# JoshuaQSH/FALCON-TTDforGNNs

Hardware: AMD Instinct MI355X
Metric: tt_embedding_lookups_per_sec (higher is better)
Workload: dtype f32; 1 GPU; ogbn-products TTEmbeddingBag fwd+bwd+SGD per step, frontier of a 2048-seed batch = 409600 unique uniform ids per GPU, bag length 1; num_embeddings=2449029, ids_per_gpu_step=409600, parallelism=dp1

## Files before the change

### falcon-ttdforgnns_amd/csrc/ttemb_api.hip

```cpp
#include "ttemb_common.h"
#include "ttemb_cache.h"

#include <dlfcn.h>

#include <atomic>
#include <cstdarg>
#include <cstdio>
#include <cstdlib>
#include <cstring>

namespace ttemb {

static thread_local char g_err[512] = "";
static std::atomic<int> g_path{TTEMB_PATH_AUTO};

int fail(int code, const char* fmt, ...) {
  va_list ap;
  va_start(ap, fmt);
  vsnprintf(g_err, sizeof(g_err), fmt, ap);
  va_end(ap);
  return code;
}

int check_hip(hipError_t e, const char* what) {
// ... 930 lines not shown

extern "C" {

int ttemb_abi_version(void) { return TTEMB_ABI_VERSION; }

const char* ttemb_last_error(void) { return g_err; }

int ttemb_set_path(int32_t path) {
  if (path < TTEMB_PATH_AUTO || path > TTEMB_PATH_PER_BAG) return fail(TTEMB_E_BADARG, "unknown path %d", path);
  g_path.store(path);
  return TTEMB_OK;
}

int ttemb_set_piece_limits(int64_t rows, int64_t ids) {
  fast3_set_piece_limits(rows, ids);
  return TTEMB_OK;
}

int ttemb_set_wide_slab_min_ids(int64_t ids) {
  fast3_set_wide_slab_min_ids(ids);
  return TTEMB_OK;
}

int ttemb_grouping_layout(const ttemb_shape_t* shape, int64_t nnz, int64_t* out) {
  if (shape == nullptr || out == nullptr || nnz < 0) return fail(TTEMB_E_BADARG, "grouping_layout: bad argument");
  DevShape ds;
  int rc = make_dev_shape(shape, &ds);
  if (rc) return rc;
  return fast3_grouping_layout(ds, nnz, out);
}

int ttemb_set_spin_limit(int64_t tries) {
  fast3_set_spin_limit(tries);
  return TTEMB_OK;
}

int ttemb_init(void) { return fault_word_init(); }

int ttemb_status(void) {
  if (g_fault_state.load(std::memory_order_acquire) == 0) (void)fault_word_init();
  return pending_device_fault();
}

int ttemb_profile_enable(int32_t on) {
  if (on != 0)
    for (int i = 0; i < kProfSlots; ++i) g_prof_valid[i] = false;
// ... 653 lines not shown
```

### falcon-ttdforgnns_amd/csrc/ttemb_common.h

```cpp
#pragma once

#include <hip/hip_runtime.h>
#include <stdint.h>

#include <atomic>

#include "../../include/ttemb.h"

namespace ttemb {

constexpr int kWave = 64;
constexpr int kMaxProbes = 3;
constexpr int64_t kEmptyKey = -1;

struct DevShape {
  int T;
  int p[TTEMB_MAX_CORES];
  int q[TTEMB_MAX_CORES];
  int R[TTEMB_MAX_CORES + 1];
  long long L[TTEMB_MAX_CORES];
  int D;
  int row_len[TTEMB_MAX_CORES];
  int part_len[TTEMB_MAX_CORES];
  int part_max;
// ... 19 lines not shown
};
int allow_big_lds(const void* kernel, size_t lds_bytes, LdsGate* gate, const char* what);
int device_cus();

int64_t generic_fwd_lds_bytes(const DevShape& s);
int64_t generic_bwd_lds_bytes(const DevShape& s);
int launch_forward_generic(const DevShape& s, const CorePtrs& cores, const int64_t* indices,
                           const int64_t* rowidx, const int64_t* offsets, int64_t B, int64_t nnz,
                           const int32_t* nnz_dev, float* output, hipStream_t st);
int launch_backward_generic(const DevShape& s, const CorePtrs& cores, const int64_t* indices,
                            const int64_t* rowidx, const int64_t* offsets, int64_t B, int64_t nnz,
                            const int32_t* nnz_dev, const float* d_output, const CorePtrsMut& d_cores, hipStream_t st);
int launch_zero_cores(const DevShape& s, const CorePtrsMut& d_cores, hipStream_t st);

bool fast3_supported(const DevShape& s);
bool fast3_pays(const DevShape& s, int64_t nnz);
bool fast3_prefix_in_chain(const DevShape& s, int64_t nnz, int64_t B);
bool fast3_group_products_in_chain(const DevShape& s, int64_t nnz, int64_t B);
bool fast3_fits(const DevShape& s, int64_t nnz, int64_t B);
bool fast3_fits_in_pieces(const DevShape& s, int64_t nnz, int64_t B);
void fast3_set_piece_limits(int64_t rows, int64_t ids);
int fast3_grouping_layout(const DevShape& s, int64_t nnz, int64_t* out);
void fast3_set_spin_limit(int64_t tries);
void fast3_set_wide_slab_min_ids(int64_t ids);
uint32_t* fault_word(hipStream_t st);
int fault_word_init();
int pending_device_fault();
int64_t fast3_workspace_bytes(const DevShape& s, int32_t op, int64_t nnz, int64_t B);
int64_t fast3_plan_bytes(const DevShape& s, int64_t nnz);
int launch_forward_fast3(const DevShape& s, const CorePtrs& cores, const int64_t* indices,
                         const int64_t* rowidx, const int64_t* offsets, int64_t nnz,
                         const int32_t* nnz_dev, int64_t B, float* output, bool zero_rows, void* ws,
                         int64_t ws_bytes, void* plan, int64_t plan_bytes, int phase, hipStream_t st, void* header);
constexpr int64_t kFast3HeaderBytes = 40960;
struct FusedUpdateK {
  float* w[TTEMB_MAX_CORES];
  float* st[TTEMB_MAX_CORES];
  float lr, eps;
  const float* lr_dev;
  float* v[TTEMB_MAX_CORES];
  uint32_t* step;
  float b1, omb1, b2, omb2;
  float wd;
  int32_t decoupled;
  uint32_t* poison_out;
  int32_t sticky;
// ... 128 lines not shown
```

### falcon-ttdforgnns_amd/csrc/ttemb_fast3.hip

```cpp
#include "ttemb_common.h"
#include "ttemb_cache.h"

#include <atomic>
#include <cstdlib>
#include <cstring>



namespace ttemb {

typedef float f32x4 __attribute__((ext_vector_type(4)));


constexpr int kChunk = 16;
constexpr uint32_t kMultiBit = 0x80000000u;

template <int Q0, int Q1, int Q2, int R1, int R2>
struct Cfg {
  static constexpr int M2 = Q0 * Q1;
  static constexpr int MT2 = (M2 + 15) / 16;
  static constexpr int KS1 = R1 / 4;
  static constexpr int KS2 = R2 / 4;
  static constexpr int N1 = Q1 * R2;
  static constexpr int NT1 = (N1 + 15) / 16;
// ... 2113 lines not shown
      if constexpr (SHARED) {
        for (int e0 = 0; e0 < ROW2; e0 += kWave) {
          const int e = e0 + lane, src = (e >> 2) & 63;
          const float x = __shfl(acc[n].x, src, kWave), y = __shfl(acc[n].y, src, kWave);
          const float z = __shfl(acc[n].z, src, kWave), w = __shfl(acc[n].w, src, kWave);
          const float v = (e & 3) == 0 ? x : ((e & 3) == 1 ? y : ((e & 3) == 2 ? z : w));
          if (e < ROW2) atomicAdd(slab + (size_t)i2 * stride + e, v);
        }
      } else {
        if (lane < F4) *reinterpret_cast<float4*>(slab + (size_t)i2 * stride + 4 * lane) = acc[n];
      }
    }
  }
}

#ifndef TTEMB_EPI_SLICES
#define TTEMB_EPI_SLICES 16
#endif
constexpr int kEpiSlices = TTEMB_EPI_SLICES;
__device__ __forceinline__ bool sparse_groups(const GroupPlan& plan, uint32_t G) {
  return __builtin_amdgcn_readfirstlane(plan.counts[G]) * 4u < 3u * G;
}

template <int Q0, int Q1, int Q2, int R1, int R2>
struct EpiCfg {
  static constexpr int G1_BYTES = R1 * (Q1 * R2 + 1) * 4;
#ifndef TTEMB_EPI_SHARE_BYTES
#define TTEMB_EPI_SHARE_BYTES (8 * 1024)
#endif
  static constexpr int WAVES = G1_BYTES > TTEMB_EPI_SHARE_BYTES ? 4 : 1;
};

template <int Q0, int Q1, int Q2, int R1, int R2, bool SKIP>
__device__ __forceinline__ void epilogue_unit(
    const float* __restrict__ G0, const float* __restrict__ G1, uint32_t p0, uint32_t p1, uint32_t gpw, const GroupPlan& plan,
    float* dpbuf, float* g1buf, uint32_t slice, uint32_t slices, uint32_t i1) {
  using C = Cfg<Q0, Q1, Q2, R1, R2>;
  constexpr int GM = 16 / Q0;
  constexpr int LDD = C::N1 + 4;
  constexpr int PF = C::M2 * R2;
  constexpr int BF4 = 16 * C::N1 / 4;
  constexpr int NLB = (BF4 + kWave - 1) / kWave;
  constexpr int KS3 = C::N1 / 4;
  static_assert(C::N1 % 4 == 0, "dP rows move as float4");
  constexpr int EW = EpiCfg<Q0, Q1, Q2, R1, R2>::WAVES;
  const int lane = threadIdx.x & 63;
  const int hi = lane >> 4, lo = lane & 15;
  const bool active = slice < slices;
  const uint32_t i0_begin = active ? slice * gpw : p0;
  const uint32_t i0_end = i0_begin + gpw < p0 ? i0_begin + gpw : p0;
  const uint32_t g_begin = i1 * p0 + (active ? i0_begin : 0u);
  const uint32_t G = p0 * p1;
  const rsrc_t r_dp = make_rsrc(plan.dptab, G * (uint32_t)PF * 4u);
  const rsrc_t r_g0 = make_rsrc(G0, p0 * (uint32_t)C::ROW0 * 4u);
  const rsrc_t r_part = make_rsrc(plan.g0part, G * (uint32_t)C::ROW0 * 4u);

  f32x4 g1acc[C::RT1][C::NT1];
#pragma unroll
  for (int t = 0; t < C::RT1; ++t)
#pragma unroll
    for (int nt = 0; nt < C::NT1; ++nt) g1acc[t][nt] = (f32x4){0.f, 0.f, 0.f, 0.f};

  const uint32_t cnt_l = (i0_begin + lane < i0_end) ? plan.counts[g_begin + lane] : 0u;
  const unsigned long long live = __ballot(cnt_l != 0);
  float4 nxt[NLB];
  float nxt_g0[4][C::RT1];
  auto request = [&](uint32_t k0) {
#pragma unroll
    for (int it = 0; it < NLB; ++it) {
      const int e = it * kWave + lane;
      const uint32_t gi = k0 + (uint32_t)(4 * e / PF);
      const bool on = (BF4 % kWave == 0 || e < BF4) && 4 * e / PF < GM && gi < gpw && ((live >> gi) & 1ull);
      nxt[it] = buf_load4(r_dp, on ? (g_begin + k0) * (uint32_t)(PF * 4) + 16u * e : kOob);
    }
#pragma unroll
    for (int s = 0; s < 4; ++s) {
      const int rho = 4 * s + hi;
      const uint32_t gi = k0 + (uint32_t)(rho / Q0);
      const bool on = rho / Q0 < GM && gi < gpw && ((live >> gi) & 1ull);
#pragma unroll
      for (int t = 0; t < C::RT1; ++t)
        nxt_g0[s][t] = __uint_as_float(buf_load1u(
            r_g0, (on && 16 * t + lo < R1) ? (i0_begin + gi) * (uint32_t)(C::ROW0 * 4) + 4u * ((rho % Q0) * R1 + 16 * t + lo) : kOob));
    }
  };
  auto next_live = [&](uint32_t k) {
    if constexpr (SKIP) {
      while (k < gpw && !((live >> k) & ((1ull << GM) - 1ull))) k += GM;
    }
    return k;
  };
  if constexpr (SKIP) {
    if (active && lane == 0) plan.epi_live[(size_t)slice * p1 + i1] = live != 0ull ? 1u : 0u;
    if (EW == 1 && live == 0ull) return;
  }
  const uint32_t k_first = next_live(0);
  request(k_first);
  {
    const float* g1 = G1 + (size_t)i1 * C::ROW1;
    constexpr int NG1 = (C::ROW1 + EW * kWave - 1) / (EW * kWave);
    const int t0 = (int)threadIdx.x;
    float g1v[NG1];
#pragma unroll
    for (int it = 0; it < NG1; ++it) {
      const int e = it * EW * kWave + t0;
      g1v[it] = (C::ROW1 % (EW * kWave) == 0 || e < C::ROW1) ? g1[e] : 0.f;
    }
#pragma unroll
    for (int it = 0; it < NG1; ++it) {
      const int e = it * EW * kWave + t0;
      if (C::ROW1 % (EW * kWave) == 0 || e < C::ROW1) g1buf[(e / C::N1) * C::LDG + e % C::N1] = g1v[it];
    }
    if constexpr (EW > 1) {
      __syncthreads();
      if (!active || (SKIP && live == 0ull)) return;
    }
  }
  const uint32_t n_here = i0_end - i0_begin;
  for (uint32_t k0 = k_first; k0 < n_here;) {
    float g0v[4][C::RT1];
#pragma unroll
    for (int it = 0; it < NLB; ++it) {
      const int e = it * kWave + lane;
      if (BF4 % kWave == 0 || e < BF4) *reinterpret_cast<float4*>(dpbuf + (4 * e / C::N1) * LDD + (4 * e) % C::N1) = nxt[it];
    }
#pragma unroll
    for (int s = 0; s < 4; ++s)
#pragma unroll
      for (int t = 0; t < C::RT1; ++t) g0v[s][t] = nxt_g0[s][t];
    __builtin_amdgcn_sched_barrier(0);
    const uint32_t k_next = next_live(k0 + GM);
    request(k_next);
    __builtin_amdgcn_fence(__ATOMIC_RELEASE, "wavefront");
    __builtin_amdgcn_wave_barrier();
    __builtin_amdgcn_fence(__ATOMIC_ACQUIRE, "wavefront");
    float b1[4][C::NT1];
#pragma unroll
    for (int s = 0; s < 4; ++s)
// ... 20 lines not shown
    f32x4 g0part[4][C::RT1];
#pragma unroll
    for (int c = 0; c < 4; ++c)
#pragma unroll
      for (int t = 0; t < C::RT1; ++t) g0part[c][t] = (f32x4){0.f, 0.f, 0.f, 0.f};
#pragma unroll
    for (int s = 0; s < KS3; ++s)
#pragma unroll
      for (int t = 0; t < C::RT1; ++t)
        g0part[s & 3][t] = __builtin_amdgcn_mfma_f32_16x16x4f32(a3[s], b3[s][t], g0part[s & 3][t], 0, 0, 0);
#pragma unroll
    for (int t = 0; t < C::RT1; ++t) {
      const f32x4 sum = (g0part[0][t] + g0part[1][t]) + (g0part[2][t] + g0part[3][t]);
#pragma unroll
      for (int r = 0; r < 4; ++r) {
        const int rho = 4 * hi + r;
        const uint32_t gi = k0 + (uint32_t)(rho / Q0);
        const bool on = rho / Q0 < GM && gi < n_here && 16 * t + lo < R1;
        buf_store1(r_part, on ? (g_begin + gi) * (uint32_t)(C::ROW0 * 4) + 4u * ((rho % Q0) * R1 + 16 * t + lo) : kOob, sum[r]);
      }
    }
    k0 = k_next;
  }
  float* dst = plan.g1part + ((size_t)slice * p1 + i1) * C::ROW1;
#pragma unroll
  for (int t = 0; t < C::RT1; ++t)
#pragma unroll
    for (int nt = 0; nt < C::NT1; ++nt)
#pragma unroll
      for (int r = 0; r < 4; ++r) {
        const int c = 16 * t + 4 * hi + r;
        if (c < R1 && (C::N1 % 16 == 0 || 16 * nt + lo < C::N1)) dst[c * C::N1 + 16 * nt + lo] = g1acc[t][nt][r];
      }
}

template <int Q0, int Q1, int Q2, int R1, int R2>
__global__ __launch_bounds__((EpiCfg<Q0, Q1, Q2, R1, R2>::WAVES * 64)) void fast3_group_epilogue_kernel(
    const float* __restrict__ G0, const float* __restrict__ G1, uint32_t p0, uint32_t p1, uint32_t gpw, uint32_t slices, GroupPlan plan,
    AdamPrep adam) {
  using C = Cfg<Q0, Q1, Q2, R1, R2>;
  constexpr int EW = EpiCfg<Q0, Q1, Q2, R1, R2>::WAVES;
  if (adam.step != nullptr && blockIdx.x == 0 && threadIdx.x == 0) adam_prepare(adam);
  __shared__ __attribute__((aligned(16))) float dpbuf_all[EW][16 * (C::N1 + 4)];
  __shared__ __attribute__((aligned(16))) float g1buf[R1 * C::LDG];
  const uint32_t wave = threadIdx.x >> 6;
  float* dpbuf = dpbuf_all[wave];
  const uint32_t nsb = (slices + EW - 1u) / EW;
  const uint32_t i1_blk = blockIdx.x / nsb;
  const uint32_t slice = (blockIdx.x - i1_blk * nsb) * EW + wave;
  if (sparse_groups(plan, p0 * p1))
    epilogue_unit<Q0, Q1, Q2, R1, R2, true>(G0, G1, p0, p1, gpw, plan, dpbuf, g1buf, slice, slices, i1_blk);
  else
    epilogue_unit<Q0, Q1, Q2, R1, R2, false>(G0, G1, p0, p1, gpw, plan, dpbuf, g1buf, slice, slices, i1_blk);
}

__device__ __forceinline__ void finalize_emit(const FusedUpdateK& upd, const AdamCoef& ac, float lr, int t, float* __restrict__ grad, int idx, float g) {
  if (upd.w[0] == nullptr) {
    grad[idx] = upd.eps != 0.f ? grad[idx] + g : g;
  } else if (upd.st[0] == nullptr) {
    upd.w[t][idx] -= lr * g;
  } else if (upd.v[0] != nullptr) {
    float w = upd.w[t][idx], m = upd.st[t][idx], v = upd.v[t][idx];
    adam_element(w, m, v, g, ac, lr, upd.eps, upd.b1, upd.omb1, upd.b2, upd.omb2, upd.wd, upd.decoupled);
    upd.st[t][idx] = m;
    upd.v[t][idx] = v;
    upd.w[t][idx] = w;
  } else {
    const float s2 = upd.st[t][idx] + g * g;
    upd.st[t][idx] = s2;
    upd.w[t][idx] -= lr * g / (sqrtf(s2) + upd.eps);
  }
}

__global__ __launch_bounds__(256) void fast3_finalize_kernel(GroupPlan plan, int tiles, int slices, int p0, int p1,
                                                             int g2_floats, int row0, int g1_floats, int q2, int r2,
                                                             float* __restrict__ dG0, float* __restrict__ dG1,
// ... 377 lines not shown
  const int64_t least = forced > 0 ? forced : (int64_t)8 * wide_slab_shares(s) * s.p[2];
  return nnz >= least;
}
static int64_t slab_count(const DevShape& s, int64_t nnz) {
  if (wide_slab(s, nnz)) return wide_slab_shares(s);
  return fused_dg2(s) ? fused_tiles(s, nnz) : (shared_slab(s) ? 1 : reduce_tiles(nnz));
}
static int epi_groups_per_wave(const DevShape& s) {
  int gpw = (s.p[0] + kEpiSlices - 1) / kEpiSlices;
  return gpw < 1 ? 1 : (gpw > 64 ? 64 : gpw);
}
static int wide_k_chunk(const DevShape& s) {
  const int64_t tiles = (int64_t)(s.R[1] / 64) * (s.q[1] * s.R[2] / 64) * s.p[1];
  int64_t parts = (4096 + tiles - 1) / tiles;
  parts = parts < 1 ? 1 : (parts > 8 ? 8 : parts);
  const int64_t K = (int64_t)s.p[0] * s.q[0];
  return (int)(((K + parts - 1) / parts + 31) / 32 * 32);
}
static int64_t wide_rows_stride(const DevShape& s) { return ((int64_t)s.p[0] * s.q[0] + 63) / 64 * 64 + 64; }
static int epi_slices(const DevShape& s) {
  if (wide(s)) return (int)(((int64_t)s.p[0] * s.q[0] + wide_k_chunk(s) - 1) / wide_k_chunk(s));
  const int g = epi_groups_per_wave(s);
  return (s.p[0] + g - 1) / g;
}

static int64_t max_chunks(const DevShape& s, int64_t nnz) {
  const int64_t G = num_groups(s);
  return nnz / kChunk + (nnz < G ? nnz : G) + 1;
}

int64_t fast3_plan_bytes(const DevShape& s, int64_t nnz) {
  const int64_t G = num_groups(s);
  return 2 * align256(nnz * 4) + align256((G + 1) * 4) + align256((G + 3) * 8) + align256(max_chunks(s, nnz) * 16) +
         align256(G * (int64_t)s.q[0] * s.q[1] * s.R[2] * 4);
}

static void carve_plan_part(const DevShape& s, int64_t nnz, char* base, GroupPlan* pl) {
  const int64_t G = num_groups(s);
  pl->i2s = (uint32_t*)base;
  base += align256(nnz * 4);
  pl->vals = (uint32_t*)base;
  base += align256(nnz * 4);
  pl->counts = (uint32_t*)base;
  base += align256((G + 1) * 4);
  pl->gpre = (uint64_t*)base;
  base += align256((G + 3) * 8);
// ... 422 lines not shown
#endif
    rc = run_wide_gemm<true, true, 1>(g, s, plan, st, "wide3_gemm_kernel (dG0)");
    if (rc) return rc;
  }
  {
    const int g2_floats = s.p[2] * C::ROW2, g1_floats = s.p[1] * C::ROW1;
    const int wgs = (g2_floats + 31) / 32 + (s.p[0] * C::ROW0 + 31) / 32 + (g1_floats + 1023) / 1024;
    hipLaunchKernelGGL(fast3_finalize_kernel, dim3((unsigned)wgs), dim3(256), 0, st, plan, (int)slab_count(s, nnz), epi_slices(s), s.p[0], s.p[1],
                       g2_floats, (int)C::ROW0, g1_floats, Q2, R2, d_cores.c[0], d_cores.c[1], d_cores.c[2], upd, 1);
  }
  profile_end(1, st);
  return check_hip(hipGetLastError(), "fast3_finalize_kernel (wide)");
}

#ifndef TTEMB_GFUSE_IDS
#define TTEMB_GFUSE_IDS -1
#endif
constexpr int64_t kGFuseIdsPerGroup = TTEMB_GFUSE_IDS;
template <int Q0, int Q1, int Q2, int R1, int R2>
struct GFuseCfg {
  using C = Cfg<Q0, Q1, Q2, R1, R2>;
  static constexpr bool ok = 16 / Q0 >= 2 && C::N1 % 16 == 0 && Q1 > 1;
};
static int64_t gfuse_limit(const DevShape& s) {
  if (kGFuseIdsPerGroup >= 0) return kGFuseIdsPerGroup;
  return s.R[2] >= 32 ? (int64_t(1) << 40) : (s.q[0] == 8 ? 16 : 8);
}

static bool gfuse_pays(const DevShape& s, int64_t nnz) {
  if (gfuse_limit(s) <= 0 || !classify(s) || fused_dg2(s)) return false;
  bool ok = false;
#define TTEMB_X(a, b, c, d, e) if (shape_is(s, a, b, c, d, e)) ok = GFuseCfg<a, b, c, d, e>::ok;
  TTEMB_FAST3_SHAPES(TTEMB_X)
#undef TTEMB_X
  const int64_t G = num_groups(s);
  return ok && (gfuse_limit(s) >= (int64_t(1) << 40) || nnz < gfuse_limit(s) * G) && (uint64_t)G * (uint64_t)s.p[0] < (uint64_t(1) << 40);
}
bool fast3_group_products_in_chain(const DevShape& s, int64_t nnz, int64_t B) { return fits_piece(s, nnz, B) && gfuse_pays(s, nnz); }

template <int Q0, int Q1, int Q2, int R1, int R2>
static int run_backward(const DevShape& s, const CorePtrs& cores, const GroupPlan& plan, int64_t nnz, int64_t B,
                        const float* d_output, const CorePtrsMut& d_cores, const FusedUpdate& upd, hipStream_t st) {
  using C = Cfg<Q0, Q1, Q2, R1, R2>;
  const int64_t G = num_groups(s);
  profile_begin(1, st);
  int rc;
  constexpr size_t wave_lds = (size_t)(C::PB_FLOATS + C::BB2_FLOATS + C::OB_FLOATS) * sizeof(float);
// ... 54 lines not shown
                       (uint32_t)G, (uint32_t)s.p[2], (uint32_t)nnz, d_output, (uint32_t)(B * s.D * 4), plan, GroupFuse{});
    profile_end(2, st);
    rc = check_hip(hipGetLastError(), "fast3_bwd_chunk_kernel");
    if (rc) return rc;
  }
  const int tiles = (int)reduce_tiles(nnz);
  const size_t reduce_lds = (size_t)(2 * s.p[2] + 1) * 4 + kRowsB * 2;
  const AdamPrep no_adam{nullptr, 0.0, 0.0};
  const AdamPrep reduce_adam = gfuse ? adam_prep_of(upd) : no_adam, epi_adam = gfuse ? no_adam : adam_prep_of(upd);
  if (fused) {
  } else if (shared_slab(s)) {
    rc = launch_zero(plan.g2part, (size_t)s.p[2] * C::ROW2 * 4, st, "zero the shared dG2 slab");
    if (rc) return rc;
    hipLaunchKernelGGL((fast3_dg2_reduce_kernel<C::ROW2, kRowsB, NWB, true>), dim3((unsigned)tiles), dim3(NWB * 64), reduce_lds, st,
                       plan, (int)G, (uint32_t)s.p[2], (uint32_t)reduce_rows(nnz), (uint32_t)C::ROW2, reduce_adam);

  } else {
    hipLaunchKernelGGL((fast3_dg2_reduce_kernel<C::ROW2, kRowsB, NWB, false>), dim3((unsigned)tiles), dim3(NWB * 64), reduce_lds, st,
                       plan, (int)G, (uint32_t)s.p[2], (uint32_t)reduce_rows(nnz), (uint32_t)C::ROW2, reduce_adam);
  }
  rc = check_hip(hipGetLastError(), "fast3_dg2_reduce_kernel");
  if (rc) return rc;
  const int gpw = epi_groups_per_wave(s), slices = gfuse ? 1 : epi_slices(s);
  if (!gfuse) {
    constexpr int EW = EpiCfg<Q0, Q1, Q2, R1, R2>::WAVES;
    const unsigned epi_blocks = (unsigned)((slices + EW - 1) / EW) * (unsigned)s.p[1];
    profile_begin(8, st);
#if defined(TTEMB_ABL) && (TTEMB_ABL & 512)
    if (fused)
#endif
    hipLaunchKernelGGL((fast3_group_epilogue_kernel<Q0, Q1, Q2, R1, R2>), dim3(epi_blocks),
                       dim3(EW * 64), 0, st, cores.c[0], cores.c[1], (uint32_t)s.p[0], (uint32_t)s.p[1], (uint32_t)gpw, (uint32_t)slices, plan,
                       epi_adam);
    profile_end(8, st);
    rc = check_hip(hipGetLastError(), "fast3_group_epilogue_kernel");
    if (rc) return rc;
  }
  {
    const int g2_floats = s.p[2] * C::ROW2, g1_floats = s.p[1] * C::ROW1;
    const int wgs = (g2_floats + 31) / 32 + (s.p[0] * C::ROW0 + 31) / 32 + (g1_floats + 1023) / 1024;
    profile_begin(9, st);
    hipLaunchKernelGGL(fast3_finalize_kernel, dim3((unsigned)wgs), dim3(256), 0, st, plan, (int)slab_count(s, nnz), slices,
                       s.p[0], s.p[1], g2_floats, (int)C::ROW0, g1_floats, Q2, R2, d_cores.c[0], d_cores.c[1], d_cores.c[2], upd, gfuse ? (kPartsByI0 ? 3 : 1) : 0);
    profile_end(9, st);
  }
  profile_end(1, st);
  return check_hip(hipGetLastError(), "fast3_finalize_kernel");
}

__global__ __launch_bounds__(64) void window_piece_kernel(const int64_t* __restrict__ offsets, long long bag0, long long B, int D,
                                                          Piece* __restrict__ out) {
  if (blockIdx.x != 0 || threadIdx.x != 0) return;
  Piece pc;
  pc.pos0 = (long long)offsets[bag0];
  pc.count = (long long)offsets[bag0 + B] - pc.pos0;
  if (pc.count < 0) pc.count = 0;
  pc.rowbase = bag0;
  pc.zero0 = bag0;
  pc.zero1 = bag0 + B;
  pc.window_bytes = B * (long long)D * 4;
  *out = pc;
}
constexpr int64_t kWindowHeadBytes = 256;
bool fast3_window_fits(const DevShape& s, int64_t nnz, int64_t bags_total, int64_t B) {
  return fits_shape(s) && (classify(s) || wide(s)) && nnz > 0 && B > 0 && fits_piece(s, nnz, B) && bags_total < 0x7fffffffll;
// ... 164 lines not shown
```

### falcon-ttdforgnns_amd/ttemb_native.py

```python
from __future__ import annotations

import ctypes
import os
from typing import List, Optional, Sequence

import torch

_HERE = os.path.dirname(os.path.abspath(__file__))
LIB_PATH = os.environ.get("TTEMB_LIB") or os.path.join(_HERE, "lib", "libttemb_hip.so")

MAX_CORES = 4
ABI_VERSION = 4
OP_FORWARD, OP_BACKWARD, OP_PREPROCESS, OP_CACHE_POPULATE = 0, 1, 2, 3
PATH_AUTO, PATH_GENERIC, PATH_FAST3, PATH_PER_BAG = 0, 1, 2, 3

EXPORTED_SYMBOLS = (
    "ttemb_abi_version", "ttemb_last_error", "ttemb_workspace_bytes", "ttemb_plan_bytes", "ttemb_set_path",
    "ttemb_profile_enable", "ttemb_profile_read", "ttemb_kernel_family", "ttemb_set_piece_limits", "ttemb_set_wide_slab_min_ids", "ttemb_init", "ttemb_status", "ttemb_set_spin_limit", "ttemb_grouping_layout",
    "ttemb_forward", "ttemb_forward_group", "ttemb_forward_lookup", "ttemb_backward_dense", "ttemb_backward_sgd", "ttemb_backward_adagrad",
    "ttemb_window_workspace_bytes", "ttemb_forward_window", "ttemb_backward_dense_window", "ttemb_backward_sgd_window", "ttemb_backward_adagrad_window",
    "ttemb_sgd_step", "ttemb_sgd_step_guarded", "ttemb_adagrad_step", "ttemb_cache_update", "ttemb_cache_update_one_sweep", "ttemb_cache_populate",
    "ttemb_preprocess", "ttemb_preprocess_update", "ttemb_cache_forward", "ttemb_cache_backward_sgd",
    "ttemb_cache_backward_dense", "ttemb_cache_backward_rowwise_adagrad",
    "ttemb_exact_workspace_bytes", "ttemb_exact_plan_bytes", "ttemb_set_exact_grid", "ttemb_forward_exact",
    "ttemb_backward_dense_exact", "ttemb_backward_sgd_exact", "ttemb_backward_adagrad_exact",
    "ttemb_bag_workspace_bytes", "ttemb_bag_reduce", "ttemb_bag_reduce_backward", "ttemb_bag_mean",
    "ttemb_drop_padding_workspace_bytes", "ttemb_drop_padding", "ttemb_pad_weights",
    "ttemb_backward_adam", "ttemb_backward_adam_window", "ttemb_backward_adam_exact", "ttemb_adam_step",
    "ttemb_bag_max_workspace_bytes", "ttemb_bag_max", "ttemb_bag_max_backward",
    "ttemb_stage_call",
    "ttemb_backward_step", "ttemb_backward_step_window", "ttemb_backward_step_exact", "ttemb_flat_step",
)

BAGS_SYMBOLS = ("ttemb_stage_bags", "ttemb_bag_reduce_n", "ttemb_bag_reduce_backward_n", "ttemb_bag_max_n",
                "ttemb_bag_max_backward_n", "ttemb_pad_weights_n")



class Shape(ctypes.Structure):
    _fields_ = [("T", ctypes.c_int32), ("p", ctypes.c_int32 * MAX_CORES),
                ("q", ctypes.c_int32 * MAX_CORES), ("R", ctypes.c_int32 * (MAX_CORES + 1))]


class AdamParams(ctypes.Structure):
    _fields_ = [("lr", ctypes.c_float), ("eps", ctypes.c_float), ("weight_decay", ctypes.c_float),
                ("decoupled", ctypes.c_int32), ("beta1", ctypes.c_double), ("beta2", ctypes.c_double)]


class StepDesc(ctypes.Structure):
    _fields_ = [("kind", ctypes.c_int32), ("lr_dev", ctypes.c_void_p), ("eps", ctypes.c_float), ("state", ctypes.c_void_p),
                ("state2", ctypes.c_void_p), ("adam_step", ctypes.c_void_p), ("adam", ctypes.c_void_p)]


STEP_SGD, STEP_ADAGRAD, STEP_ADAM = 0, 1, 2

# ... 66 lines not shown
def _load() -> ctypes.CDLL:
    if not os.path.exists(LIB_PATH):
        raise ImportError(
            f"{LIB_PATH} is missing: build it with `python -c 'import __graft_entry__ as g; g.build()'` "
            "or `make -C falcon-ttdforgnns_amd/csrc`.  There is no CPU fallback for the TT embedding path.")
    lib = ctypes.CDLL(LIB_PATH)
    vp, i64, i32, f32 = ctypes.c_void_p, ctypes.c_int64, ctypes.c_int32, ctypes.c_float
    shp = ctypes.POINTER(Shape)
    lib.ttemb_abi_version.restype = ctypes.c_int
    if lib.ttemb_abi_version() != ABI_VERSION:
        raise ImportError(f"{LIB_PATH}: ABI version {lib.ttemb_abi_version()}, this binding needs {ABI_VERSION} -- rebuild the library "
                          "(`make -C falcon-ttdforgnns_amd/csrc`)")
    lib.ttemb_last_error.restype = ctypes.c_char_p
    lib.ttemb_workspace_bytes.restype = i64
    lib.ttemb_workspace_bytes.argtypes = [shp, i32, i64, i64]
    lib.ttemb_set_path.argtypes = [i32]
    lib.ttemb_profile_enable.argtypes = [i32]
    lib.ttemb_profile_read.argtypes = [i32, ctypes.POINTER(ctypes.c_float)]
    lib.ttemb_kernel_family.argtypes = [shp, i64, i64, i32]
    lib.ttemb_set_piece_limits.argtypes = [i64, i64]
    lib.ttemb_set_spin_limit.argtypes = [i64]
    lib.ttemb_grouping_layout.argtypes = [shp, i64, ctypes.POINTER(ctypes.c_int64)]
    lib.ttemb_set_wide_slab_min_ids.argtypes = [i64]
    lib.ttemb_status.argtypes = []
    lib.ttemb_init.argtypes = []
    lib.ttemb_plan_bytes.restype = i64
    lib.ttemb_plan_bytes.argtypes = [shp, i64]
    lib.ttemb_forward.argtypes = [shp, vp, vp, vp, vp, i64, vp, i64, vp, vp, i64, vp, i64, vp]
    lib.ttemb_forward_group.argtypes = lib.ttemb_forward.argtypes
    lib.ttemb_forward_lookup.argtypes = lib.ttemb_forward.argtypes
    lib.ttemb_backward_dense.argtypes = [shp, vp, vp, vp, vp, i64, vp, i64, vp, vp, vp, i64, vp, i64, vp]
    lib.ttemb_backward_sgd.argtypes = [shp, vp, vp, vp, vp, i64, vp, i64, vp, f32, vp, i64, vp, i64, vp]
    lib.ttemb_backward_adagrad.argtypes = [shp, vp, vp, vp, vp, vp, i64, vp, i64, vp, f32, f32, vp, i64, vp, i64, vp]
    lib.ttemb_window_workspace_bytes.restype = i64
    lib.ttemb_window_workspace_bytes.argtypes = [shp, i32, i64, i64, i64]
    lib.ttemb_forward_window.argtypes = [shp, vp, vp, vp, i64, i64, i64, i64, vp, vp, i64, vp]
    lib.ttemb_backward_dense_window.argtypes = [shp, vp, vp, vp, i64, i64, i64, i64, vp, vp, vp, i64, vp]
    lib.ttemb_backward_sgd_window.argtypes = [shp, vp, vp, vp, i64, i64, i64, i64, vp, f32, vp, i64, vp]
    lib.ttemb_backward_adagrad_window.argtypes = [shp, vp, vp, vp, vp, i64, i64, i64, i64, vp, f32, f32, vp, i64, vp]
    lib.ttemb_sgd_step.argtypes = [vp, vp, i64, f32, vp]
    lib.ttemb_sgd_step_guarded.argtypes = [vp, vp, i64, f32, vp, vp]
    lib.ttemb_adagrad_step.argtypes = [vp, vp, vp, i64, f32, f32, vp]
    lib.ttemb_cache_update.argtypes = [vp, i64, vp, vp, i64, vp]
    lib.ttemb_cache_update_one_sweep.argtypes = [vp, i64, vp, vp, i64, vp]
    lib.ttemb_cache_populate.argtypes = [shp, vp, vp, vp, vp, i64, vp, i64, vp, i64, vp]
    lib.ttemb_preprocess.argtypes = [vp, vp, i64, i64, i32, vp, vp, i64, vp, vp, vp, vp, vp, i32, vp, i64, vp]
# ... 21 lines not shown
    lib.ttemb_bag_reduce.argtypes = [vp, vp, vp, i64, i64, i64, vp, vp, i64, vp]
    lib.ttemb_bag_reduce_backward.argtypes = [vp, vp, vp, vp, i64, i64, i64, vp, vp, vp, i64, vp]
    lib.ttemb_bag_mean.argtypes = [vp, vp, vp, i64, i64, vp]
    lib.ttemb_bag_max_workspace_bytes.restype = i64
    lib.ttemb_bag_max_workspace_bytes.argtypes = [i64, i64, i64]
    lib.ttemb_bag_max.argtypes = [vp, vp, i64, vp, i64, i64, i64, vp, vp, vp, i64, vp]
    lib.ttemb_bag_max_backward.argtypes = [vp, vp, vp, i64, i64, i64, vp, vp]
    lib.ttemb_drop_padding_workspace_bytes.restype = i64
    lib.ttemb_drop_padding_workspace_bytes.argtypes = [i64, i64]
    lib.ttemb_drop_padding.argtypes = [vp, vp, i64, i64, i64, vp, vp, vp, vp, vp, i64, vp]
    lib.ttemb_pad_weights.argtypes = [vp, vp, vp, i64, i64, i64, i32, vp, vp]
    lib.ttemb_stage_call.argtypes = [vp, i32, i64, vp, i32, i64, vp, i64, vp, i64, vp, vp]
    lib.ttemb_stage_bags.argtypes = [vp, i32, i64, vp, i32, i64, i64, vp, vp, i64, vp, i64, vp, vp, vp]
    lib.ttemb_bag_reduce_n.argtypes = [vp, vp, vp, i64, vp, i64, i64, vp, vp, i64, vp]
    lib.ttemb_bag_reduce_backward_n.argtypes = [vp, vp, vp, vp, i64, vp, i64, i64, vp, vp, vp, i64, vp]
    lib.ttemb_bag_max_n.argtypes = [vp, vp, i64, vp, i64, vp, i64, i64, vp, vp, vp, i64, vp]
    lib.ttemb_bag_max_backward_n.argtypes = [vp, vp, vp, i64, vp, i64, i64, vp, vp]
    lib.ttemb_pad_weights_n.argtypes = [vp, vp, vp, i64, vp, i64, i64, i32, vp, vp]
    stp = ctypes.POINTER(StepDesc)
    lib.ttemb_backward_step.argtypes = [shp, vp, vp, vp, vp, i64, vp, i64, vp, stp, vp, i64, vp, i64, vp]
    lib.ttemb_backward_step_window.argtypes = [shp, vp, vp, vp, i64, i64, i64, i64, vp, stp, vp, i64, vp]
    lib.ttemb_backward_step_exact.argtypes = [shp, vp, vp, vp, i64, i64, vp, stp, vp, i64, vp, i64, vp]
    lib.ttemb_flat_step.argtypes = [vp, vp, vp, vp, vp, i64, f32, stp, vp, vp]
    for name in EXPORTED_SYMBOLS + BAGS_SYMBOLS:
        fn = getattr(lib, name)
        if name not in ("ttemb_last_error", "ttemb_workspace_bytes", "ttemb_plan_bytes", "ttemb_window_workspace_bytes",
                        "ttemb_exact_workspace_bytes", "ttemb_exact_plan_bytes", "ttemb_bag_workspace_bytes",
                        "ttemb_drop_padding_workspace_bytes", "ttemb_bag_max_workspace_bytes"):
            fn.restype = ctypes.c_int
    return lib


LIB = _load()
_STEP_FN = {family: tuple(getattr(LIB, "ttemb_backward_" + kind + suffix) for kind in ("sgd", "adagrad", "adam", "step"))
            for family, suffix in (("plain", ""), ("window", "_window"), ("exact", "_exact"))}
_STEP_FN["flat"] = (LIB.ttemb_sgd_step, LIB.ttemb_adagrad_step, LIB.ttemb_adam_step, LIB.ttemb_flat_step)


def _check(rc: int) -> None:
    if rc != 0:
        raise RuntimeError(f"libttemb_hip: {LIB.ttemb_last_error().decode()} (status {rc})")


def _ptr(t: Optional[torch.Tensor]) -> Optional[int]:
    if t is None:
        return None
    if not t.is_cuda:
# ... 174 lines not shown
    _check(LIB.ttemb_set_spin_limit(tries))


def status() -> None:
    _check(LIB.ttemb_status())


def grouping_layout(shape: Shape, nnz: int) -> dict:
    out = (ctypes.c_int64 * 5)()
    _check(LIB.ttemb_grouping_layout(ctypes.byref(shape), nnz, out))
    return dict(zip(("slices", "ranges", "banks", "cap", "ovf_slots"), (int(x) for x in out)))


def set_piece_limits(rows: int = 0, ids: int = 0) -> None:
    global path_epoch
    _check(LIB.ttemb_set_piece_limits(rows, ids))
    _size_cache.clear()
    path_epoch += 1


def set_wide_slab_min_ids(ids: int = 0) -> None:
    global path_epoch
    _check(LIB.ttemb_set_wide_slab_min_ids(ids))
    _size_cache.clear()
    path_epoch += 1


def new_plan(shape: Shape, nnz: int, device: torch.device) -> Optional[torch.Tensor]:
    n = plan_bytes(shape, nnz)
    return torch.empty(n, dtype=torch.uint8, device=device) if n > 0 else None


def _plan_args(plan: Optional[torch.Tensor]):
    return (None, 0) if plan is None else (plan.data_ptr(), plan.numel())


def forward(shape: Shape, cores: Sequence[torch.Tensor], indices: torch.Tensor, rowidx: torch.Tensor,
            offsets: Optional[torch.Tensor], nnz: int, nnz_dev: Optional[torch.Tensor], B: int,
            output: torch.Tensor, ws: Workspace, plan: Optional[torch.Tensor] = None, phase: int = 0) -> None:
    dev = output.device
    w = ws.get(workspace_bytes(shape, OP_FORWARD, nnz, B), dev)
    fn = (LIB.ttemb_forward, LIB.ttemb_forward_group, LIB.ttemb_forward_lookup)[phase]
    with _on_device(dev):
        _check(fn(ctypes.byref(shape), _ptr_array(cores), _ptr(indices), _ptr(rowidx),
                  _ptr(offsets), nnz, _ptr(nnz_dev), B, _ptr(output), _ptr(w), w.numel(),
                  *_plan_args(plan), _stream(output)))
# ... 589 lines not shown
```

### include/ttemb.h

```cpp
#ifndef TTEMB_H_
#define TTEMB_H_

#include <stdint.h>

#ifdef __cplusplus
extern "C" {
#endif

#define TTEMB_ABI_VERSION 4
#define TTEMB_MAX_CORES 4

enum {
  TTEMB_OK = 0,
  TTEMB_E_BADARG = -1,
  TTEMB_E_WORKSPACE = -2,
  TTEMB_E_UNSUPPORTED = -3,
  TTEMB_E_HIP = -4
};

typedef struct ttemb_shape {
  int32_t T;
  int32_t p[TTEMB_MAX_CORES];
  int32_t q[TTEMB_MAX_CORES];
  int32_t R[TTEMB_MAX_CORES + 1];
// ... 226 lines not shown
                              float* d_weights , void* workspace, int64_t workspace_bytes,
                              void* stream);
int ttemb_bag_mean(const float* src, float* dst, const int64_t* offsets, int64_t B, int64_t D, void* stream);

int64_t ttemb_bag_max_workspace_bytes(int64_t nnz, int64_t B, int64_t D);
int ttemb_bag_max(const float* rows, const int64_t* indices , int64_t pad, const int64_t* offsets,
                  int64_t nnz, int64_t B, int64_t D, float* output, int32_t* argmax, void* workspace, int64_t workspace_bytes,
                  void* stream);
int ttemb_bag_max_backward(const float* d_output, const int32_t* argmax, const int64_t* offsets, int64_t nnz, int64_t B,
                           int64_t D, float* d_rows, void* stream);

int64_t ttemb_drop_padding_workspace_bytes(int64_t nnz, int64_t B);
int ttemb_drop_padding(const int64_t* indices, const int64_t* offsets, int64_t nnz, int64_t B, int64_t pad,
                       int64_t* indices_out, int64_t* rowidx_out, int64_t* offsets_out, int32_t* nnz_kept_dev, void* workspace,
                       int64_t workspace_bytes, void* stream);
int ttemb_pad_weights(const int64_t* indices, const int64_t* offsets, const float* weights, int64_t nnz, int64_t B,
                      int64_t pad, int32_t mean, float* weights_out, void* stream);

#ifdef __cplusplus
}
#endif

#include "ttemb_bags.h"

#endif
```

Baseline: 2.196 billion lookups/s.

## Reduce epilogue dG1 partials across waves in LDS before writing slabs

The group epilogue now sizes its wave count from an LDS budget and uses dynamic shared memory. Each workgroup's waves sum their dG1 accumulators in LDS and write one partial per slab instead of one per slice. This shrinks the g1part traffic and the work left for the finalize kernel, at the cost of extra barriers and possibly lower occupancy from the larger LDS footprint. A diagnostic setter to force the group-products threshold is also added.

New measurement: 2.195 billion lookups/s (median of 2 runs). About the same (-0.1%).

```diff
diff --git a/falcon-ttdforgnns_amd/csrc/ttemb_api.hip b/falcon-ttdforgnns_amd/csrc/ttemb_api.hip
--- a/falcon-ttdforgnns_amd/csrc/ttemb_api.hip
+++ b/falcon-ttdforgnns_amd/csrc/ttemb_api.hip
@@ -976,6 +976,11 @@
   return TTEMB_OK;
 }
 
+int ttemb_set_group_products_ids(int64_t ids_per_group) {
+  fast3_set_group_products_ids(ids_per_group);
+  return TTEMB_OK;
+}
+
 int ttemb_grouping_layout(const ttemb_shape_t* shape, int64_t nnz, int64_t* out) {
   if (shape == nullptr || out == nullptr || nnz < 0) return fail(TTEMB_E_BADARG, "grouping_layout: bad argument");
   DevShape ds;
diff --git a/falcon-ttdforgnns_amd/csrc/ttemb_common.h b/falcon-ttdforgnns_amd/csrc/ttemb_common.h
--- a/falcon-ttdforgnns_amd/csrc/ttemb_common.h
+++ b/falcon-ttdforgnns_amd/csrc/ttemb_common.h
@@ -65,6 +65,7 @@
 void fast3_set_piece_limits(int64_t rows, int64_t ids);
 int fast3_grouping_layout(const DevShape& s, int64_t nnz, int64_t* out);
 void fast3_set_spin_limit(int64_t tries);
+void fast3_set_group_products_ids(int64_t ids);
 void fast3_set_wide_slab_min_ids(int64_t ids);
 uint32_t* fault_word(hipStream_t st);
 int fault_word_init();
diff --git a/falcon-ttdforgnns_amd/csrc/ttemb_fast3.hip b/falcon-ttdforgnns_amd/csrc/ttemb_fast3.hip
--- a/falcon-ttdforgnns_amd/csrc/ttemb_fast3.hip
+++ b/falcon-ttdforgnns_amd/csrc/ttemb_fast3.hip
@@ -2159,19 +2159,31 @@
   return __builtin_amdgcn_readfirstlane(plan.counts[G]) * 4u < 3u * G;
 }
 
+#ifndef TTEMB_EPI_WAVES
+#define TTEMB_EPI_WAVES 4
+#endif
+constexpr int epi_lds_floats(int q1, int r1, int r2, int ew) {
+  return ew * 16 * (q1 * r2 + 4) + r1 * (q1 * r2 + 1) + ew;
+}
+constexpr int epi_waves_of(int q1, int r1, int r2) {
+  int ew = TTEMB_EPI_WAVES;
+  while (ew > 1 && (size_t)epi_lds_floats(q1, r1, r2, ew) * 4 > kCuLds) ew /= 2;
+  return ew;
+}
 template <int Q0, int Q1, int Q2, int R1, int R2>
 struct EpiCfg {
-  static constexpr int G1_BYTES = R1 * (Q1 * R2 + 1) * 4;
-#ifndef TTEMB_EPI_SHARE_BYTES
-#define TTEMB_EPI_SHARE_BYTES (8 * 1024)
-#endif
-  static constexpr int WAVES = G1_BYTES > TTEMB_EPI_SHARE_BYTES ? 4 : 1;
+  static constexpr int WAVES = epi_waves_of(Q1, R1, R2);
+  static constexpr int LDS_FLOATS = epi_lds_floats(Q1, R1, R2, WAVES);
+  static constexpr int ROW1 = R1 * Q1 * R2;
+  static constexpr int PARKED = WAVES * ROW1 <= LDS_FLOATS - WAVES ? WAVES : WAVES / 2;
+  static_assert(WAVES == 1 || (WAVES & (WAVES - 1)) == 0, "the wavefronts fold by halves");
+  static_assert(WAVES == 1 || PARKED * ROW1 <= LDS_FLOATS - WAVES, "the parked dG1 copies must fit the workgroup's LDS");
 };
 
 template <int Q0, int Q1, int Q2, int R1, int R2, bool SKIP>
 __device__ __forceinline__ void epilogue_unit(
     const float* __restrict__ G0, const float* __restrict__ G1, uint32_t p0, uint32_t p1, uint32_t gpw, const GroupPlan& plan,
-    float* dpbuf, float* g1buf, uint32_t slice, uint32_t slices, uint32_t i1) {
+    float* lds, float* dpbuf, float* g1buf, uint32_t slice, uint32_t slices, uint32_t i1) {
   using C = Cfg<Q0, Q1, Q2, R1, R2>;
   constexpr int GM = 16 / Q0;
   constexpr int LDD = C::N1 + 4;
@@ -2180,9 +2192,11 @@
   constexpr int NLB = (BF4 + kWave - 1) / kWave;
   constexpr int KS3 = C::N1 / 4;
   static_assert(C::N1 % 4 == 0, "dP rows move as float4");
-  constexpr int EW = EpiCfg<Q0, Q1, Q2, R1, R2>::WAVES;
+  using E = EpiCfg<Q0, Q1, Q2, R1, R2>;
+  constexpr int EW = E::WAVES;
   const int lane = threadIdx.x & 63;
   const int hi = lane >> 4, lo = lane & 15;
+  const uint32_t slab = slice / EW;
   const bool active = slice < slices;
   const uint32_t i0_begin = active ? slice * gpw : p0;
   const uint32_t i0_end = i0_begin + gpw < p0 ? i0_begin + gpw : p0;
@@ -2227,9 +2241,9 @@
     }
     return k;
   };
-  if constexpr (SKIP) {
-    if (active && lane == 0) plan.epi_live[(size_t)slice * p1 + i1] = live != 0ull ? 1u : 0u;
-    if (EW == 1 && live == 0ull) return;
+  if constexpr (SKIP && EW == 1) {
+    if (lane == 0) plan.epi_live[(size_t)slab * p1 + i1] = live != 0ull ? 1u : 0u;
+    if (live == 0ull) return;
   }
   const uint32_t k_first = next_live(0);
   request(k_first);
@@ -2248,9 +2262,15 @@
       const int e = it * EW * kWave + t0;
       if (C::ROW1 % (EW * kWave) == 0 || e < C::ROW1) g1buf[(e / C::N1) * C::LDG + e % C::N1] = g1v[it];
     }
-    if constexpr (EW > 1) {
+    if constexpr (EW > 1 && SKIP) {
+      uint32_t* has_ids = reinterpret_cast<uint32_t*>(lds + E::LDS_FLOATS - EW);
+      if (lane == 0) has_ids[threadIdx.x >> 6] = live != 0ull ? 1u : 0u;
       __syncthreads();
-      if (!active || (SKIP && live == 0ull)) return;
+      const bool any = __ballot(lane < EW && has_ids[lane < EW ? lane : 0] != 0u) != 0ull;
+      if (threadIdx.x == 0) plan.epi_live[(size_t)slab * p1 + i1] = any ? 1u : 0u;
+      if (!any) return;
+    } else if constexpr (EW > 1) {
+      __syncthreads();
     }
   }
   const uint32_t n_here = i0_end - i0_begin;
@@ -2317,16 +2337,52 @@
     }
     k0 = k_next;
   }
-  float* dst = plan.g1part + ((size_t)slice * p1 + i1) * C::ROW1;
-#pragma unroll
-  for (int t = 0; t < C::RT1; ++t)
-#pragma unroll
-    for (int nt = 0; nt < C::NT1; ++nt)
-#pragma unroll
-      for (int r = 0; r < 4; ++r) {
-        const int c = 16 * t + 4 * hi + r;
-        if (c < R1 && (C::N1 % 16 == 0 || 16 * nt + lo < C::N1)) dst[c * C::N1 + 16 * nt + lo] = g1acc[t][nt][r];
-      }
+  float* dst = plan.g1part + ((size_t)slab * p1 + i1) * C::ROW1;
+#ifdef TTEMB_EPI_ABL_NO_SLABS
+  if (p0 != 0xffffffffu) return;
+#endif
+  auto park = [&](int slot, bool add) {
+    float* cp = lds + slot * C::ROW1;
+    if constexpr (EW == 1) cp = dst;
+#pragma unroll
+    for (int t = 0; t < C::RT1; ++t)
+#pragma unroll
+      for (int nt = 0; nt < C::NT1; ++nt)
+#pragma unroll
+        for (int r = 0; r < 4; ++r) {
+          const int c = 16 * t + 4 * hi + r;
+          if (c < R1 && (C::N1 % 16 == 0 || 16 * nt + lo < C::N1)) {
+            float* e = cp + c * C::N1 + 16 * nt + lo;
+            if (add) g1acc[t][nt][r] += *e;
+            else *e = g1acc[t][nt][r];
+          }
+        }
+  };
+  if constexpr (EW == 1) {
+    park(0, false);
+  } else {
+    const int wave = (int)(threadIdx.x >> 6);
+    __syncthreads();
+    if constexpr (E::PARKED < EW) {
+      if (wave >= E::PARKED) park(wave - E::PARKED, false);
+      __syncthreads();
+      if (wave < E::PARKED) park(wave, true);
+      __syncthreads();
+    }
+    if (wave < E::PARKED) park(wave, false);
+    __syncthreads();
+    constexpr int F4 = C::ROW1 / 4;
+    const float4* cp4 = reinterpret_cast<const float4*>(lds);
+    for (int e = (int)threadIdx.x; e < F4; e += EW * kWave) {
+      float4 s = cp4[e];
+#pragma unroll
+      for (int w = 1; w < E::PARKED; ++w) {
+        const float4 v = cp4[w * F4 + e];
+        s.x += v.x; s.y += v.y; s.z += v.z; s.w += v.w;
+      }
+      *reinterpret_cast<float4*>(dst + 4 * e) = s;
+    }
+  }
 }
 
 template <int Q0, int Q1, int Q2, int R1, int R2>
@@ -2336,17 +2392,18 @@
   using C = Cfg<Q0, Q1, Q2, R1, R2>;
   constexpr int EW = EpiCfg<Q0, Q1, Q2, R1, R2>::WAVES;
   if (adam.step != nullptr && blockIdx.x == 0 && threadIdx.x == 0) adam_prepare(adam);
-  __shared__ __attribute__((aligned(16))) float dpbuf_all[EW][16 * (C::N1 + 4)];
-  __shared__ __attribute__((aligned(16))) float g1buf[R1 * C::LDG];
+  extern __shared__ __attribute__((aligned(16))) float smem[];
+  static_assert((16 * (C::N1 + 4)) % 4 == 0 && C::LDG == C::N1 + 1, "epi_lds_floats() describes this layout");
   const uint32_t wave = threadIdx.x >> 6;
-  float* dpbuf = dpbuf_all[wave];
+  float* dpbuf = smem + wave * (16 * (C::N1 + 4));
+  float* g1buf = smem + EW * (16 * (C::N1 + 4));
   const uint32_t nsb = (slices + EW - 1u) / EW;
   const uint32_t i1_blk = blockIdx.x / nsb;
   const uint32_t slice = (blockIdx.x - i1_blk * nsb) * EW + wave;
   if (sparse_groups(plan, p0 * p1))
-    epilogue_unit<Q0, Q1, Q2, R1, R2, true>(G0, G1, p0, p1, gpw, plan, dpbuf, g1buf, slice, slices, i1_blk);
+    epilogue_unit<Q0, Q1, Q2, R1, R2, true>(G0, G1, p0, p1, gpw, plan, smem, dpbuf, g1buf, slice, slices, i1_blk);
   else
-    epilogue_unit<Q0, Q1, Q2, R1, R2, false>(G0, G1, p0, p1, gpw, plan, dpbuf, g1buf, slice, slices, i1_blk);
+    epilogue_unit<Q0, Q1, Q2, R1, R2, false>(G0, G1, p0, p1, gpw, plan, smem, dpbuf, g1buf, slice, slices, i1_blk);
 }
 
 __device__ __forceinline__ void finalize_emit(const FusedUpdateK& upd, const AdamCoef& ac, float lr, int t, float* __restrict__ grad, int idx, float g) {
@@ -2770,6 +2827,11 @@
   if (wide(s)) return (int)(((int64_t)s.p[0] * s.q[0] + wide_k_chunk(s) - 1) / wide_k_chunk(s));
   const int g = epi_groups_per_wave(s);
   return (s.p[0] + g - 1) / g;
+}
+static int epi_slabs(const DevShape& s) {
+  if (wide(s)) return epi_slices(s);
+  const int ew = epi_waves_of(s.q[1], s.R[1], s.R[2]);
+  return (epi_slices(s) + ew - 1) / ew;
 }
 
 static int64_t max_chunks(const DevShape& s, int64_t nnz) {
@@ -3238,7 +3300,11 @@
   using C = Cfg<Q0, Q1, Q2, R1, R2>;
   static constexpr bool ok = 16 / Q0 >= 2 && C::N1 % 16 == 0 && Q1 > 1;
 };
+static std::atomic<int64_t> g_gfuse_ids{-1};
+void fast3_set_group_products_ids(int64_t ids) { g_gfuse_ids.store(ids < 0 ? -1 : ids); }
 static int64_t gfuse_limit(const DevShape& s) {
+  const int64_t forced = g_gfuse_ids.load();
+  if (forced >= 0) return forced;
   if (kGFuseIdsPerGroup >= 0) return kGFuseIdsPerGroup;
   return s.R[2] >= 32 ? (int64_t(1) << 40) : (s.q[0] == 8 ? 16 : 8);
 }
@@ -3339,15 +3405,26 @@
   rc = check_hip(hipGetLastError(), "fast3_dg2_reduce_kernel");
   if (rc) return rc;
   const int gpw = epi_groups_per_wave(s), slices = gfuse ? 1 : epi_slices(s);
+#ifdef TTEMB_EPI_ABL_NO_SLABS
+  const int slabs = 1;
+#else
+  const int slabs = gfuse ? 1 : epi_slabs(s);
+#endif
   if (!gfuse) {
-    constexpr int EW = EpiCfg<Q0, Q1, Q2, R1, R2>::WAVES;
+    using E = EpiCfg<Q0, Q1, Q2, R1, R2>;
+    constexpr int EW = E::WAVES;
+    if (EW != epi_waves_of(s.q[1], s.R[1], s.R[2])) return fail(TTEMB_E_HIP, "internal: epi_slabs() and EpiCfg out of step");
     const unsigned epi_blocks = (unsigned)((slices + EW - 1) / EW) * (unsigned)s.p[1];
+    constexpr size_t epi_lds = (size_t)E::LDS_FLOATS * sizeof(float);
+    static LdsGate epi_lds_ok;
+    rc = allow_big_lds(reinterpret_cast<const void*>(fast3_group_epilogue_kernel<Q0, Q1, Q2, R1, R2>), epi_lds, &epi_lds_ok, "group epilogue kernel");
+    if (rc) return rc;
     profile_begin(8, st);
 #if defined(TTEMB_ABL) && (TTEMB_ABL & 512)
     if (fused)
 #endif
     hipLaunchKernelGGL((fast3_group_epilogue_kernel<Q0, Q1, Q2, R1, R2>), dim3(epi_blocks),
-                       dim3(EW * 64), 0, st, cores.c[0], cores.c[1], (uint32_t)s.p[0], (uint32_t)s.p[1], (uint32_t)gpw, (uint32_t)slices, plan,
+                       dim3(EW * 64), epi_lds, st, cores.c[0], cores.c[1], (uint32_t)s.p[0], (uint32_t)s.p[1], (uint32_t)gpw, (uint32_t)slices, plan,
                        epi_adam);
     profile_end(8, st);
     rc = check_hip(hipGetLastError(), "fast3_group_epilogue_kernel");
@@ -3357,7 +3434,7 @@
     const int g2_floats = s.p[2] * C::ROW2, g1_floats = s.p[1] * C::ROW1;
     const int wgs = (g2_floats + 31) / 32 + (s.p[0] * C::ROW0 + 31) / 32 + (g1_floats + 1023) / 1024;
     profile_begin(9, st);
-    hipLaunchKernelGGL(fast3_finalize_kernel, dim3((unsigned)wgs), dim3(256), 0, st, plan, (int)slab_count(s, nnz), slices,
+    hipLaunchKernelGGL(fast3_finalize_kernel, dim3((unsigned)wgs), dim3(256), 0, st, plan, (int)slab_count(s, nnz), slabs,
                        s.p[0], s.p[1], g2_floats, (int)C::ROW0, g1_floats, Q2, R2, d_cores.c[0], d_cores.c[1], d_cores.c[2], upd, gfuse ? (kPartsByI0 ? 3 : 1) : 0);
     profile_end(9, st);
   }
diff --git a/falcon-ttdforgnns_amd/ttemb_native.py b/falcon-ttdforgnns_amd/ttemb_native.py
--- a/falcon-ttdforgnns_amd/ttemb_native.py
+++ b/falcon-ttdforgnns_amd/ttemb_native.py
@@ -31,6 +31,8 @@
     "ttemb_stage_call",
     "ttemb_backward_step", "ttemb_backward_step_window", "ttemb_backward_step_exact", "ttemb_flat_step",
 )
+
+DIAG_SYMBOLS = ("ttemb_set_group_products_ids",)
 
 BAGS_SYMBOLS = ("ttemb_stage_bags", "ttemb_bag_reduce_n", "ttemb_bag_reduce_backward_n", "ttemb_bag_max_n",
                 "ttemb_bag_max_backward_n", "ttemb_pad_weights_n")
@@ -143,6 +145,7 @@
     lib.ttemb_set_spin_limit.argtypes = [i64]
     lib.ttemb_grouping_layout.argtypes = [shp, i64, ctypes.POINTER(ctypes.c_int64)]
     lib.ttemb_set_wide_slab_min_ids.argtypes = [i64]
+    lib.ttemb_set_group_products_ids.argtypes = [i64]
     lib.ttemb_status.argtypes = []
     lib.ttemb_init.argtypes = []
     lib.ttemb_plan_bytes.restype = i64
@@ -210,7 +213,7 @@
     lib.ttemb_backward_step_window.argtypes = [shp, vp, vp, vp, i64, i64, i64, i64, vp, stp, vp, i64, vp]
     lib.ttemb_backward_step_exact.argtypes = [shp, vp, vp, vp, i64, i64, vp, stp, vp, i64, vp, i64, vp]
     lib.ttemb_flat_step.argtypes = [vp, vp, vp, vp, vp, i64, f32, stp, vp, vp]
-    for name in EXPORTED_SYMBOLS + BAGS_SYMBOLS:
+    for name in EXPORTED_SYMBOLS + BAGS_SYMBOLS + DIAG_SYMBOLS:
         fn = getattr(lib, name)
         if name not in ("ttemb_last_error", "ttemb_workspace_bytes", "ttemb_plan_bytes", "ttemb_window_workspace_bytes",
                         "ttemb_exact_workspace_bytes", "ttemb_exact_plan_bytes", "ttemb_bag_workspace_bytes",
@@ -431,6 +434,13 @@
 def set_wide_slab_min_ids(ids: int = 0) -> None:
     global path_epoch
     _check(LIB.ttemb_set_wide_slab_min_ids(ids))
+    _size_cache.clear()
+    path_epoch += 1
+
+
+def set_group_products_ids(ids_per_group: int = -1) -> None:
+    global path_epoch
+    _check(LIB.ttemb_set_group_products_ids(ids_per_group))
     _size_cache.clear()
     path_epoch += 1
 
diff --git a/include/ttemb.h b/include/ttemb.h
--- a/include/ttemb.h
+++ b/include/ttemb.h
@@ -272,5 +272,6 @@
 #endif
 
 #include "ttemb_bags.h"
+#include "ttemb_diag.h"
 
 #endif
diff --git a/include/ttemb_diag.h b/include/ttemb_diag.h
--- /dev/null
+++ b/include/ttemb_diag.h
@@ -0,0 +1,16 @@
+#ifndef TTEMB_DIAG_H_
+#define TTEMB_DIAG_H_
+
+#include <stdint.h>
+
+#ifdef __cplusplus
+extern "C" {
+#endif
+
+int ttemb_set_group_products_ids(int64_t ids_per_group);
+
+#ifdef __cplusplus
+}
+#endif
+
+#endif
```
